# oppo-us-research/PoP-Net

Hardware: AMD Instinct MI355X
Metric: depth-frames/sec end-to-end (480x640) (higher is better)
Workload: dtype bf16

## Files before the change

### popnet_amd/csrc/api.hip

```cpp
#pragma clang fp contract(off)
#include <cmath>
#include <cstdio>
#include <cstdlib>
#include <cstring>
#include "pn_internal.h"
#include "preproc_pixel.h"

template <typename TIN>
__global__ void preprocess_kernel(const TIN *__restrict__ depth, float *__restrict__ out, int B, int H, int W, int S,
                                  double scale_x, double scale_y, float dmax, float mean, float stdv) {
    const unsigned pix = blockIdx.x * blockDim.x + threadIdx.x;
    if (pix >= (unsigned)(S * S)) return;
    const int b = blockIdx.y;
    const int dy = (int)(pix / (unsigned)S);
    const int dx = (int)(pix - (unsigned)dy * (unsigned)S);
    const size_t gid = (size_t)b * S * S + pix;

    out[gid] = pn_preproc_pixel(depth + (size_t)b * H * W, H, W, dy, dx, scale_x, scale_y, dmax, mean, stdv);
}

PnSwitches pn_read_switches() {
    auto set = [](const char *name) { return getenv(name) != nullptr; };
    auto num = [](const char *name, int unset) { const char *e = getenv(name); return e ? atoi(e) : unset; };
    auto is = [](const char *name, const char *value) { const char *e = getenv(name); return e && !strcmp(e, value); };
    PnSwitches s;
    s.no_conv3 = set("POPNET_NO_CONV3");
    s.conv3_rpg8 = set("POPNET_CONV3_RPG8");
    s.conv3_pt14 = num("POPNET_CONV3_PT14", 0);
    s.conv3_nbuf2 = set("POPNET_CONV3_NBUF2");
    s.generic_c64_off = num("POPNET_GENERIC_C64", 1) == 0;
    if (set("POPNET_CONV4")) s.conv4 = num("POPNET_CONV4", 0) == 0 ? 0 : 1;
    s.no_mix = set("POPNET_NO_MIX");
    s.no_bblock = set("POPNET_NO_BBLOCK");
    s.bblock_x3 = num("POPNET_BBLOCK_X3", 0) != 0;
    s.bb64_static = set("POPNET_BB64_STATIC");
    s.bb64_halves = num("POPNET_BB64_HALVES", 1) == 2 ? 2 : 1;
    s.no_tailfuse = set("POPNET_NO_TAILFUSE");
    s.no_poolfuse = set("POPNET_NO_POOLFUSE");
    s.no_stempool = set("POPNET_NO_STEMPOOL");
    s.no_embed3 = set("POPNET_NO_EMBED3");
    s.train_x3_wide = set("POPNET_TRAIN_X3_WIDE");
    s.train_wgrad_novec = set("POPNET_TRAIN_WGRAD_NOVEC");
    s.trainx_one_stream = num("POPNET_TRAINX_STREAMS", 0) == 1;
    s.trainx_stem_handover = set("POPNET_TRAINX_STEM_HANDOVER");
    s.trainx_stem_gather = is("POPNET_TRAINX_STEM_FWD", "gather");
    s.trainx_stem_bn_separate = is("POPNET_TRAINX_STEM_BN", "separate");
    s.trainx_stem_depth = num("POPNET_TRAINX_STEM_DEPTH", 2);
    s.trainx_pack_gather = is("POPNET_TRAINX_PACK", "gather");
    s.trainx_legacy_wgrad = is("POPNET_TRAINX_WGRAD", "legacy");
    return s;
}

extern "C" {

int pn_abi_version(void) { return PN_ABI_VERSION; }
int pn_build_experiments(void) { return 0; }

pn_ctx *pn_create(int device_id) {
    pn_ctx *ctx = new pn_ctx();
    ctx->device = device_id;
    int ndev = 0;
    hipError_t e = hipGetDeviceCount(&ndev);
    if (e != hipSuccess || device_id < 0 || device_id >= ndev) {
        char buf[256];
        snprintf(buf, sizeof buf, "pn_create: device %d not available (%d devices, %s)", device_id, ndev,
                 hipGetErrorString(e));
        ctx->err = buf;
        ctx->device = -1;
        return ctx;
    }
    hipDeviceProp_t prop;
    if (hipGetDeviceProperties(&prop, device_id) == hipSuccess) ctx->num_cus = prop.multiProcessorCount;
    return ctx;
}

void pn_destroy(pn_ctx *ctx) {
    if (!ctx) return;
    if (ctx->parse_ws) (void)hipFree(ctx->parse_ws);
    pn_parse_big_free(ctx);
    if (ctx->train_ws) (void)hipFree(ctx->train_ws);
    for (void *p : ctx->train_ws_retired) (void)hipFree(p);
    for (auto &e : ctx->train_packs) (void)hipFree(e.buf);
    if (ctx->train_pack_table) (void)hipFree(ctx->train_pack_table);
    delete ctx;
}

int pn_last_error(pn_ctx *ctx, char *buf, size_t buf_len) {
    if (!ctx) return 0;
    if (buf && buf_len) {
        size_t n = ctx->err.size() < buf_len - 1 ? ctx->err.size() : buf_len - 1;
        memcpy(buf, ctx->err.data(), n);
// ... 49 lines not shown
```

### popnet_amd/csrc/conv3_kernel.h

```cpp
#pragma once
#include "conv_mfma_kernel.h"

constexpr int PN_CONV3_OCC = 4;
constexpr int PN_CONV3_FAST_EPILOGUE = 2;

__device__ __forceinline__ void pn_glds16(gcptr src, unsigned lds_dst) {
    unsigned keep;
    asm volatile("s_mov_b32 %0, m0\n\ts_mov_b32 m0, %2\n\ts_nop 0\n\tglobal_load_lds_dwordx4 %1, off\n\ts_mov_b32 m0, %0"
                 : "=&s"(keep) : "v"(src), "s"(lds_dst) : "memory");
}

template <int IMM>
__device__ __forceinline__ void pn_glds16_s(const void *sbase, unsigned voff, unsigned lds_dst) {
    unsigned keep;
    asm volatile("s_mov_b32 %0, m0\n\ts_mov_b32 m0, %3\n\ts_nop 0\n\tglobal_load_lds_dwordx4 %1, %2 offset:%4\n\ts_mov_b32 m0, %0"
                 : "=&s"(keep) : "v"(voff), "s"(sbase), "s"(lds_dst), "n"(IMM) : "memory");
}

typedef __attribute__((ext_vector_type(2))) unsigned int u32x2;

template <int KS, int WC, int WP, int NBUF, int PT, int RPG = PT * 4 / 7, int TAIL = 0>
__device__ __forceinline__ void conv3_body(const ConvProblem &P) {
    typedef __bf16 T;
    typedef Elem<PN_PREC_BF16>::Frag Frag;
// ... 403 lines not shown
                    if (cw + k < cout) np[(size_t)k * hw] = v[k];
            }
        }
    };
#define PN3_PIXOF(ba) ((unsigned)(ba) >> 6)
    const int wave_c0 = (cb * WC + wc) * (CT * 16);
    const bool fast = (PN_CONV3_FAST_EPILOGUE == 1 || (PN_CONV3_FAST_EPILOGUE == 2 && WC == 4)) &&
                      wave_c0 + CT * 16 <= cout && P.out && !nchw && !split && !res_split && (act == PN_ACT_RELU || act == PN_ACT_LEAKY || act == PN_ACT_NONE);
    auto finish_fast = [&](auto actc, auto resc) {
        constexpr int ACT = decltype(actc)::value;
        constexpr bool RES = decltype(resc)::value;
        PN_GLOBAL T *ob = (PN_GLOBAL T *)P.out + P.out_coff + wave_c0;
        const PN_GLOBAL T *rb = (const PN_GLOBAL T *)P.res + P.res_coff + wave_c0;
        const unsigned lane_c = (unsigned)(LC * q);
        int ba[PT];
#pragma clang loop unroll(full)
        for (int pt = 0; pt < PT; ++pt) { ba[pt] = baddr[pt]; asm volatile("" : "+v"(ba[pt])); }
        u32x4 rq[PT];
        if (RES) {
#pragma clang loop unroll(full)
            for (int pt = 0; pt < PT; ++pt) {
                const unsigned t = PN3_PIXOF(ba[pt]);
                const unsigned opix = (unsigned)pix0 + (t >> 5) * (unsigned)Wo + (t & 31u);
                rq[pt] = *reinterpret_cast<const PN_GLOBAL u32x4 *>(rb + (opix * (unsigned)res_cs + lane_c));
            }
        }
#pragma clang loop unroll(full)
        for (int pt = 0; pt < PT; ++pt) {
            const int slot = (wp * PT + pt) * 16 + c;
            const unsigned t = PN3_PIXOF(ba[pt]);
            const unsigned opix = (unsigned)pix0 + (t >> 5) * (unsigned)Wo + (t & 31u);
            float v[LC];
#pragma unroll
            for (int ct = 0; ct < CT; ++ct)
#pragma unroll
                for (int i = 0; i < 4; ++i) v[4 * ct + i] = acc[ct][pt][i] + bias[4 * ct + i];
            if (RES) {
                T rv[LC];
                *reinterpret_cast<u32x4 *>(rv) = rq[pt];
#pragma unroll
                for (int k = 0; k < LC; ++k) v[k] += (float)rv[k];
            }
#pragma unroll
            for (int k = 0; k < LC; ++k) {
                if (ACT == PN_ACT_RELU) v[k] = v[k] > 0.f ? v[k] : 0.f;
                else if (ACT == PN_ACT_LEAKY) v[k] = v[k] > 0.f ? v[k] : v[k] * 0.1f;
            }
            T ov[LC];
#pragma unroll
            for (int k = 0; k < LC; ++k) ov[k] = (T)v[k];
            if (slot < npix) *reinterpret_cast<PN_GLOBAL u32x4 *>(ob + (opix * (unsigned)out_cs + lane_c)) = *reinterpret_cast<u32x4 *>(ov);
        }
    };
    if (fast) {
        if (P.res) {
            if (act == PN_ACT_RELU) finish_fast(std::integral_constant<int, PN_ACT_RELU>{}, std::true_type{});
            else if (act == PN_ACT_LEAKY) finish_fast(std::integral_constant<int, PN_ACT_LEAKY>{}, std::true_type{});
            else finish_fast(std::integral_constant<int, PN_ACT_NONE>{}, std::true_type{});
        } else {
            if (act == PN_ACT_RELU) finish_fast(std::integral_constant<int, PN_ACT_RELU>{}, std::false_type{});
            else if (act == PN_ACT_LEAKY) finish_fast(std::integral_constant<int, PN_ACT_LEAKY>{}, std::false_type{});
            else finish_fast(std::integral_constant<int, PN_ACT_NONE>{}, std::false_type{});
        }
        return;
    }
    if (act == PN_ACT_RELU) finish(std::integral_constant<int, PN_ACT_RELU>{});
    else if (act == PN_ACT_LEAKY) finish(std::integral_constant<int, PN_ACT_LEAKY>{});
    else if (act == PN_ACT_NONE) finish(std::integral_constant<int, PN_ACT_NONE>{});
    else finish(std::integral_constant<int, -1>{});
}

template <int KS, int WC, int WP, int NBUF, int PT, int RPG = PT * 4 / 7, int TAIL = 0>
__global__ __launch_bounds__(WC * WP * 64, PT == 14 ? 2 : (NBUF == 2 ? 3 : PN_CONV3_OCC)) void conv3_kernel(const ConvProblem *__restrict__ probs) {
    conv3_body<KS, WC, WP, NBUF, PT, RPG, TAIL>(probs[blockIdx.y]);
}

template <int UNUSED = 0>
__global__ __launch_bounds__(256, PN_CONV3_OCC) void conv3_mix_kernel(const ConvProblem *__restrict__ probs) {
    const ConvProblem &P = probs[blockIdx.y];
    if (P.tail_w) conv3_body<1, 4, 1, 1, 7, 4, 1>(P);
    else if (P.ks == 1) conv3_body<1, 4, 1, 1, 7, 4, 0>(P);
    else conv3_body<3, 4, 1, 1, 7, 4, 0>(P);
}

template <int KS, int WC, int WP, int NBUF, int PT = 7, int RPG = PT * 4 / 7, int TAIL = 0>
static int conv3_launch_one(pn_ctx *ctx, const ConvLaunch &L, hipStream_t stream) {
    auto kern = conv3_kernel<KS, WC, WP, NBUF, PT, RPG, TAIL>;
    if (L.lds_bytes > 48 * 1024) {
        static PnLdsAttr attr;
        if (int rc = pn_lds_attr(ctx, attr, reinterpret_cast<const void *>(kern), L.lds_bytes)) return rc;
    }
    hipLaunchKernelGGL(kern, dim3(L.max_blocks, L.nprob), dim3(WC * WP * 64), L.lds_bytes, stream, L.probs_dev);
    PN_HIP_CHECK(ctx, hipGetLastError());
    return PN_OK;
}
#define PN3_CASE(KS, WC, WP, NB) \
    if (!L.mix && L.ks == KS && L.wc == WC && L.wp == WP && L.nbuf == NB && L.pt == 7 && L.rpg == 4 && !L.tail) return conv3_launch_one<KS, WC, WP, NB>(ctx, L, stream);
#define PN3_CASE_TAIL(KS, WC, WP, NB) \
    if (L.ks == KS && L.wc == WC && L.wp == WP && L.nbuf == NB && L.pt == 7 && L.rpg == 4 && L.tail == 1) return conv3_launch_one<KS, WC, WP, NB, 7, 4, 1>(ctx, L, stream);
#define PN3_CASE_POOLTAIL(KS, WC, WP, NB) \
    if (L.ks == KS && L.wc == WC && L.wp == WP && L.nbuf == NB && L.pt == 7 && L.rpg == 8 && L.tail == 2) return conv3_launch_one<KS, WC, WP, NB, 7, 8, 2>(ctx, L, stream);
#define PN3_CASE_PT(KS, WC, WP, NB, PT_) \
    if (L.ks == KS && L.wc == WC && L.wp == WP && L.nbuf == NB && L.pt == PT_ && L.rpg == PT_ * 4 / 7) return conv3_launch_one<KS, WC, WP, NB, PT_>(ctx, L, stream);
#define PN3_CASE_RPG(KS, WC, WP, NB, RPG_) \
    if (L.ks == KS && L.wc == WC && L.wp == WP && L.nbuf == NB && L.pt == 7 && L.rpg == RPG_) return conv3_launch_one<KS, WC, WP, NB, 7, RPG_>(ctx, L, stream);
int pn_launch_conv3_part0(pn_ctx *ctx, const ConvLaunch &L, hipStream_t stream);
int pn_launch_conv3_part1(pn_ctx *ctx, const ConvLaunch &L, hipStream_t stream);
int pn_launch_conv3_part2(pn_ctx *ctx, const ConvLaunch &L, hipStream_t stream);
```

### popnet_amd/csrc/net.hip

```cpp
#include <cmath>
#include <cstdarg>
#include <cstdio>
#include <algorithm>
#include <cstdlib>
#include <cstring>
#include <map>
#include <memory>
#include <vector>
#include "pn_internal.h"
#include "conv_plan.h"
#include "preproc_pixel.h"

namespace {

struct HostTensor {
    std::vector<int64_t> shape;
    std::vector<float> data;
    size_t numel() const { return data.size(); }
};

struct Buf {
    void *p = nullptr;
    int H = 0, W = 0, C = 0;
    int plane = 0;
};

struct ConvSpec {
    std::string w;
    std::string bn;
    int ks = 3, stride = 1;
    int in_buf = -1, in_coff = 0, cin = 0;
    std::vector<int> cin_map;
    int out_buf = -1, out_coff = 0;
    int res_buf = -1, res_coff = 0;
    int act = PN_ACT_NONE;
    int nchw_slot = -1;
    int cout = 0;
    int cfg = 0, pitch = 0, R = 0, Wt = 0, cin_chunks = 0;
    int kern = 0, wc = 0, wp = 0, nbuf = 0, pt = 7, rpg = 4;
    int wc_min = 0, nbuf_min = 0;
    int k4_level = 0;
    void *wpack = nullptr;
    float *bias = nullptr;
    double flops = 0;
    int tail_conv = -1;
    bool fused_away = false;
    void *tail_wpack = nullptr;
    float *tail_bias = nullptr;
    bool embed3 = false;
    bool pool_tail = false;
    int pool_out_buf = -1, pool_out_coff = 0;
};

struct Step {
    enum Type { STEM, POOL, CONV, BBLOCK } type;
    int bb_a = -1, bb_b = -1, bb_wt = 0;
    void *bb_wpack = nullptr;
    float *bb_bias1 = nullptr, *bb_bias2 = nullptr;
    int *bb_tickets = nullptr;
    bool bb_static = false;
    int bb_halves = 1;
    int out_buf = -1;
    int stem_pool_buf = -1;
    float *stem_w = nullptr, *stem_b = nullptr;
    void *stem_wfrag = nullptr;
    int stem_cin = 1;
    float *stem_scratch = nullptr;
    int mode = 0, in_buf = -1, C = 0, out_coff = 0;
    std::vector<int> conv_ids;
    ConvLaunch launch;
    std::vector<ConvProblem> host_probs;
    ConvProblem *dev_probs = nullptr;
};

uint16_t f32_to_bf16(float f) {
    uint32_t u;
    memcpy(&u, &f, 4);
    if ((u & 0x7fffffffu) > 0x7f800000u) return (uint16_t)((u >> 16) | 0x40);
    u += 0x7fffu + ((u >> 16) & 1u);
    return (uint16_t)(u >> 16);
}

}

struct pn_net {
    pn_ctx *ctx = nullptr;
    int kind = 0, num_parts = 15, a = 14, input_dim = 1;
    std::map<std::string, HostTensor> tensors;
    bool finalized = false;
    int prec = PN_PREC_F32, max_batch = 0, in_h = 0, in_w = 0;
    PnSwitches sw;
    std::vector<Buf> bufs;
    std::vector<ConvSpec> convs;
    std::vector<Step> steps;
    std::vector<void *> dev_allocs;
    float *nchw_ptr[4] = {nullptr, nullptr, nullptr, nullptr};
    int last_B = -1;
    bool x3 = false;
    bool locked = false;
    bool tickets_suspect = false;
    float *last_nchw[4] = {nullptr, nullptr, nullptr, nullptr};
    std::map<std::string, std::pair<int, std::pair<int, int>>> named;
    std::map<std::string, int> named_plane;
    double flops_per_frame = 0;
// ... 444 lines not shown
            }
            if (readers != 1 || other_reader) continue;
            ConvSpec &b = n->convs[ib];
            if (std::find(levels[li + 1].begin(), levels[li + 1].end(), ib) == levels[li + 1].end()) continue;
            const HostTensor *wb = find_t(n, b.w + ".weight");
            if (!wb || wb->shape.size() != 4 || b.ks != 1 || b.stride != 1 || wb->shape[1] != 128 || wb->shape[0] > 32 || !b.bn.empty() || b.res_buf >= 0 || b.in_coff != 0 ||
                (b.act != PN_ACT_NONE && b.act != PN_ACT_SIG && b.act != PN_ACT_SIG_PM2) ||
                !b.cin_map.empty())
                continue;
            a.tail_conv = ib;
            b.fused_away = true;
            a.flops += b.flops;
            levels[li + 1].erase(std::find(levels[li + 1].begin(), levels[li + 1].end(), ib));
        }
    }
    levels.erase(std::remove_if(levels.begin(), levels.end(), [](const std::vector<int> &l) { return l.empty(); }), levels.end());
}


void fuse_pool_tails(pn_net *n, std::vector<std::vector<int>> &levels) {
    if (n->prec != PN_PREC_BF16 || n->sw.no_poolfuse || n->sw.no_conv3) return;
    for (size_t li = 0; li + 1 < levels.size(); ++li) {
        if (levels[li].size() != 1 || levels[li][0] < 0) continue;
        const std::vector<int> &pl = levels[li + 1];
        if (pl.empty() || pl[0] != -1 || pl[1] != 0) continue;
        ConvSpec &a = n->convs[levels[li][0]];
        if (a.kern != 3 || a.ks != 1 || a.stride != 1 || a.cout != 128 || a.wc != 4 || a.wp != 1 || a.res_buf >= 0 || a.nchw_slot >= 0 || a.out_buf < 0 || a.out_coff != 0 ||
            a.tail_conv >= 0 || (a.act != PN_ACT_NONE && a.act != PN_ACT_RELU && a.act != PN_ACT_LEAKY))
            continue;
        if (pl[2] != a.out_buf || pl[4] != 128 || (pl[5] & 7)) continue;
        bool other_reader = false, rewritten = false;
        for (size_t lj = li + 2; lj < levels.size() && !rewritten; ++lj) {
            if (levels[lj].empty()) continue;
            if (levels[lj][0] == -1) {
                if (levels[lj][2] == a.out_buf) other_reader = true;
                if (levels[lj][3] == a.out_buf) rewritten = true;
                continue;
            }
            for (size_t k = levels[lj][0] == -2 ? 1 : 0; k < levels[lj].size(); ++k) {
                const ConvSpec &c = n->convs[levels[lj][k]];
                if (c.in_buf == a.out_buf || c.res_buf == a.out_buf) other_reader = true;
            }
            for (size_t k = levels[lj][0] == -2 ? 1 : 0; k < levels[lj].size(); ++k)
                if (n->convs[levels[lj][k]].out_buf == a.out_buf) rewritten = true;
        }
        if (other_reader) continue;
        a.pool_tail = true;
        a.pool_out_buf = pl[3]; a.pool_out_coff = pl[5];
        a.rpg = 8; a.nbuf = 1;
        levels.erase(levels.begin() + li + 1);
    }
}

int pack_tail(pn_net *n, ConvSpec &a) {
    pn_ctx *ctx = n->ctx;
    const ConvSpec &b = n->convs[a.tail_conv];
    const HostTensor *w = find_t(n, b.w + ".weight"), *bias = find_t(n, b.w + ".bias");
    const int cout = (int)w->shape[0];
    std::vector<uint16_t> pk((size_t)2 * 4 * 64 * 8, 0);
    for (int t = 0; t < 2; ++t)
        for (int ks = 0; ks < 4; ++ks)
            for (int lane = 0; lane < 64; ++lane) {
                const int co = pn_conv_row_channel(t, lane & 15, 2), q = lane >> 4;
                for (int j = 0; j < 8; ++j) {
                    const int ci = ks * 32 + 8 * q + j;
                    pk[(((size_t)t * 4 + ks) * 64 + lane) * 8 + j] = f32_to_bf16(co < cout ? w->data[(size_t)co * 128 + ci] : 0.f);
                }
            }
    if (int rc = dev_alloc(n, &a.tail_wpack, pk.size() * 2, false)) return rc;
    PN_HIP_CHECK(ctx, hipMemcpy(a.tail_wpack, pk.data(), pk.size() * 2, hipMemcpyHostToDevice));
    std::vector<float> hb(32, 0.f);
    for (int o = 0; o < cout; ++o) hb[o] = bias ? bias->data[o] : 0.f;
    if (int rc = dev_alloc(n, (void **)&a.tail_bias, 32 * 4, false)) return rc;
    PN_HIP_CHECK(ctx, hipMemcpy(a.tail_bias, hb.data(), 32 * 4, hipMemcpyHostToDevice));
    return PN_OK;
}

int build_rtpose(pn_net *n) {
    const int H = n->in_h, W = n->in_w;
    if (H % 8 || W % 8) return pn_set_error(n->ctx, PN_ERR_UNSUPPORTED, "input size must be a multiple of 8");
    const int H2 = H / 2, W2 = W / 2, H4 = H / 4, W4 = W / 4, H8 = H / 8, W8 = W / 8;
    const int J1 = n->num_parts + 1, L2 = 2 * n->a, LZ = n->a + 1;
    auto up4 = [](int v) { return (v + 3) / 4 * 4; };
    const int off_paf = 128, off_heat = up4(off_paf + L2), off_z = up4(off_heat + J1);
    const int cat_c = (off_z + LZ + 63) / 64 * 64;
    n->out_h = H8; n->out_w = W8;

    int A1 = new_buf(n, H2, W2, 64), A2 = new_buf(n, H2, W2, 64), T1 = new_buf(n, H2, W2, 64);
    int P1 = new_buf(n, H4, W4, 64), T2 = new_buf(n, H4, W4, 128), D2 = new_buf(n, H4, W4, 128);
    int A3 = new_buf(n, H4, W4, 128), A4 = new_buf(n, H4, W4, 128);
    int CAT = new_buf(n, H8, W8, cat_c);
    int BLa = new_buf(n, H8, W8, 256), BLb = new_buf(n, H8, W8, 256), BLc = new_buf(n, H8, W8, 128);
    int BSa = new_buf(n, H8, W8, 128), BSb = new_buf(n, H8, W8, 128);
    int BDa = new_buf(n, H8, W8, 128), BDb = new_buf(n, H8, W8, 64), BDc = new_buf(n, H8, W8, 64);
    n->named["feat"] = {CAT, {0, 128}};
    n->named["paf1"] = {CAT, {off_paf, L2}};
    n->named["heat1"] = {CAT, {off_heat, J1}};
    n->named["z1"] = {CAT, {off_z, LZ}};

    if (int rc = add_stem(n, A1)) return rc;
    std::vector<std::vector<int>> levels;
    auto level = [&](std::vector<int> ids) { levels.push_back(ids); return 0; };
    level({add_conv(n, "model0.layer1.0.conv1", "model0.layer1.0.bn1", 3, 1, A1, 0, T1, 0, PN_ACT_RELU)});
    level({add_conv(n, "model0.layer1.0.conv2", "model0.layer1.0.bn2", 3, 1, T1, 0, A2, 0, PN_ACT_RELU, A1)});
    level({add_conv(n, "model0.layer1.1.conv1", "model0.layer1.1.bn1", 3, 1, A2, 0, T1, 0, PN_ACT_RELU)});
    level({add_conv(n, "model0.layer1.1.conv2", "model0.layer1.1.bn2", 3, 1, T1, 0, A1, 0, PN_ACT_RELU, A2)});
    levels.push_back({-1, 0, A1, P1, 64, 0});
    level({add_conv(n, "model0.layer2.0.conv1", "model0.layer2.0.bn1", 3, 1, P1, 0, T2, 0, PN_ACT_RELU),
           add_conv(n, "model0.layer2.0.downsample.0", "model0.layer2.0.downsample.1", 1, 1, P1, 0, D2, 0, PN_ACT_NONE)});
    level({add_conv(n, "model0.layer2.0.conv2", "model0.layer2.0.bn2", 3, 1, T2, 0, A3, 0, PN_ACT_RELU, D2)});
    level({add_conv(n, "model0.conv2", "model0.bn2", 1, 1, A3, 0, A4, 0, PN_ACT_RELU)});
    levels.push_back({-1, 0, A4, CAT, 128, 0});

    std::vector<int> map2(cat_c, -1);
    for (int i = 0; i < 128; ++i) map2[i] = L2 + J1 + LZ + i;
    for (int i = 0; i < L2; ++i) map2[off_paf + i] = i;
    for (int i = 0; i < J1; ++i) map2[off_heat + i] = L2 + i;
    for (int i = 0; i < LZ; ++i) map2[off_z + i] = L2 + J1 + i;

    for (int stage = 1; stage <= 2; ++stage) {
        char p1[32], p2[32], p3[32];
        snprintf(p1, sizeof p1, "model%d_1", stage);
        snprintf(p2, sizeof p2, "model%d_2", stage);
        snprintf(p3, sizeof p3, "model%d_3", stage);
        auto nm = [](const char *p, int i) { return std::string(p) + "." + std::to_string(i); };
        std::vector<int> m = stage == 2 ? map2 : std::vector<int>();
        const bool last = stage == 2;
        level({add_conv(n, nm(p1, 0), nm(p1, 1), 3, 1, CAT, 0, BLa, 0, PN_ACT_LEAKY, -1, -1, m),
               add_conv(n, nm(p2, 0), nm(p2, 1), 3, 1, CAT, 0, BSa, 0, PN_ACT_LEAKY, -1, -1, m),
               add_conv(n, nm(p3, 0), nm(p3, 1), 3, 1, CAT, 0, BDa, 0, PN_ACT_LEAKY, -1, -1, m)});
        level({add_conv(n, nm(p1, 3), nm(p1, 4), 3, 1, BLa, 0, BLb, 0, PN_ACT_LEAKY),
               add_conv(n, nm(p2, 3), nm(p2, 4), 3, 1, BSa, 0, BSb, 0, PN_ACT_LEAKY),
               add_conv(n, nm(p3, 3), nm(p3, 4), 3, 1, BDa, 0, BDb, 0, PN_ACT_LEAKY)});
        level({add_conv(n, nm(p1, 6), nm(p1, 7), 3, 1, BLb, 0, BLa, 0, PN_ACT_LEAKY),
               add_conv(n, nm(p2, 6), nm(p2, 7), 3, 1, BSb, 0, BSa, 0, PN_ACT_LEAKY),
               add_conv(n, nm(p3, 6), nm(p3, 7), 3, 1, BDb, 0, BDc, 0, PN_ACT_LEAKY)});
        level({add_conv(n, nm(p1, 9), nm(p1, 10), 1, 1, BLa, 0, BLc, 0, PN_ACT_LEAKY),
               add_conv(n, nm(p2, 9), nm(p2, 10), 3, 1, BSa, 0, BSb, 0, PN_ACT_LEAKY),
               add_conv(n, nm(p3, 9), nm(p3, 10), 3, 1, BDc, 0, BDb, 0, PN_ACT_LEAKY)});
        level({add_conv(n, nm(p1, 12), "", 1, 1, BLc, 0, last ? -1 : CAT, off_paf, PN_ACT_SIG_PM2, -1, last ? 0 : -1),
               add_conv(n, nm(p2, 12), "", 3, 1, BSb, 0, last ? -1 : CAT, off_heat, PN_ACT_SIG, -1, last ? 1 : -1),
               add_conv(n, nm(p3, 12), "", 3, 1, BDb, 0, last ? -1 : CAT, off_z, PN_ACT_SIG_PM2, -1, last ? 2 : -1)});
    }

    for (auto &lv : levels)
        if (lv[0] >= 0) harmonize_level(n, lv);
    for (auto &cs : n->convs)
        if (int rc = prepare_conv(n, cs)) return rc;
    for (auto &cs : n->convs) n->flops_per_frame += cs.flops;
    fuse_basic_blocks(n, levels);
    fuse_1x1_tails(n, levels);
    fuse_pool_tails(n, levels);
    for (auto &cs : n->convs)
        if (cs.tail_conv >= 0)
            if (int rc = pack_tail(n, cs)) return rc;
    for (auto &lv : levels) {
        if (lv[0] == -1) add_pool(n, lv[1], lv[2], lv[3], lv[4], lv[5]);
        else if (lv[0] == -2) { if (int rc = add_bblock(n, lv[1], lv[2])) return rc; }
        else add_conv_level(n, lv);
    }
    return PN_OK;
}

int build_yolo(pn_net *n) {
    const int H = n->in_h, W = n->in_w;
    if (H % 16 || W % 16) return pn_set_error(n->ctx, PN_ERR_UNSUPPORTED, "input size must be a multiple of 16");
    const int H2 = H / 2, W2 = W / 2, H4 = H / 4, W4 = W / 4, H8 = H / 8, W8 = W / 8, H16 = H / 16, W16 = W / 16;
    n->out_h = H16; n->out_w = W16;
    int A1 = new_buf(n, H2, W2, 64);
    int X0 = new_buf(n, H4, W4, 64), X1 = new_buf(n, H4, W4, 64), XT = new_buf(n, H4, W4, 64);
    int Y0 = new_buf(n, H8, W8, 128), Y1 = new_buf(n, H8, W8, 128), YT = new_buf(n, H8, W8, 128), YD = new_buf(n, H8, W8, 128);
    int Na = new_buf(n, H8, W8, 256), Nb = new_buf(n, H8, W8, 256);
    int Ha = new_buf(n, H16, W16, 256), Hb = new_buf(n, H16, W16, 256), Hc = new_buf(n, H16, W16, 128);

    if (int rc = add_stem(n, A1)) return rc;
    std::vector<std::vector<int>> levels;
    auto level = [&](std::vector<int> ids) { levels.push_back(ids); };
    if (n->prec == PN_PREC_BF16 && !n->x3 && n->input_dim == 1 && !n->sw.no_stempool) n->steps.back().stem_pool_buf = X0;
    else levels.push_back({-1, 1, A1, X0, 64, 0});
    int cur = X0, other = X1;
    for (int i = 0; i < 3; ++i) {
        std::string p = "model0.layer1." + std::to_string(i);
        level({add_conv(n, p + ".conv1", p + ".bn1", 3, 1, cur, 0, XT, 0, PN_ACT_RELU)});
        level({add_conv(n, p + ".conv2", p + ".bn2", 3, 1, XT, 0, other, 0, PN_ACT_RELU, cur)});
        std::swap(cur, other);
    }
    {
        const bool embed = n->prec == PN_PREC_BF16 && !n->sw.no_embed3;
        const int c1 = add_conv(n, "model0.layer2.0.conv1", "model0.layer2.0.bn1", 3, 2, cur, 0, YT, 0, PN_ACT_RELU);
        const int cd = add_conv(n, "model0.layer2.0.downsample.0", "model0.layer2.0.downsample.1", embed ? 3 : 1, 2, cur, 0, YD, 0, PN_ACT_NONE);
        n->convs[cd].embed3 = embed;
        level({c1, cd});
    }
    level({add_conv(n, "model0.layer2.0.conv2", "model0.layer2.0.bn2", 3, 1, YT, 0, Y0, 0, PN_ACT_RELU, YD)});
    int yc = Y0, yo = Y1;
    for (int i = 1; i < 4; ++i) {
        std::string p = "model0.layer2." + std::to_string(i);
        level({add_conv(n, p + ".conv1", p + ".bn1", 3, 1, yc, 0, YT, 0, PN_ACT_RELU)});
        level({add_conv(n, p + ".conv2", p + ".bn2", 3, 1, YT, 0, yo, 0, PN_ACT_RELU, yc)});
        std::swap(yc, yo);
    }
    n->named["feat"] = {yc, {0, 128}};
    level({add_conv(n, "model1.0", "model1.1", 3, 1, yc, 0, Na, 0, PN_ACT_LEAKY)});
    level({add_conv(n, "model1.3", "model1.4", 3, 1, Na, 0, Nb, 0, PN_ACT_LEAKY)});
    level({add_conv(n, "model1.6", "model1.7", 3, 1, Nb, 0, Na, 0, PN_ACT_LEAKY)});
// ... 29 lines not shown
            const ConvSpec &cs = n->convs[id];
            const Buf &ib = n->bufs[cs.in_buf];
            ConvProblem P;
            memset(&P, 0, sizeof P);
            const size_t es = n->esize();
            (void)es;
            P.in = ib.p;
            P.wpack = cs.wpack;
            P.bias = cs.bias;
            P.B = B; P.H = ib.H; P.W = ib.W;
            P.Ho = (ib.H + 2 * (cs.ks / 2) - cs.ks) / cs.stride + 1;
            P.Wo = (ib.W + 2 * (cs.ks / 2) - cs.ks) / cs.stride + 1;
            P.cin_chunks = cs.cin_chunks;
            P.in_cs = ib.C; P.in_coff = cs.in_coff;
            if (n->x3 && ib.plane % 64)
                return pn_set_error(n->ctx, PN_ERR_UNSUPPORTED, "bf16x3: input plane of %d channels is not a multiple of 64 (the K loop wraps to the hi plane per 64-channel chunk)", ib.plane);
            P.in_wrap = n->x3 ? 2 * (ib.plane / 64) : (1 << 20);
            P.cout = cs.cout;
            if (cs.out_buf >= 0) { P.out = n->bufs[cs.out_buf].p; P.out_cs = n->bufs[cs.out_buf].C; P.out_coff = cs.out_coff; P.split = n->x3 ? n->bufs[cs.out_buf].plane : 0; }
            if (cs.res_buf >= 0) { P.res = n->bufs[cs.res_buf].p; P.res_cs = n->bufs[cs.res_buf].C; P.res_coff = cs.res_coff; P.res_split = n->x3 ? n->bufs[cs.res_buf].plane : 0; }
            if (cs.nchw_slot >= 0) P.out_nchw = n->nchw_ptr[cs.nchw_slot];
            P.act = cs.act;
            P.yolo_naf = 5 + 3 * n->num_parts;
            P.R = cs.R;
            P.Wt = cs.Wt;
            P.tiles_x = (P.Wo + cs.Wt - 1) / cs.Wt;
            P.tiles_per_img = ((P.Ho + cs.R - 1) / cs.R) * P.tiles_x;
            P.cout_blocks = (cs.cout + BC - 1) / BC;
            P.nblocks = B * P.tiles_per_img * P.cout_blocks;
            if (cs.kern == 4) P.nblocks = ((B * P.tiles_per_img + 1) / 2) * P.cout_blocks;
            P.ksteps = cs.cin_chunks * cs.ks * cs.ks * 2;
            P.ks = cs.ks;
            P.lds_buf_bytes = (int)pn_conv_lds_bytes(n->prec, cs.ks, cs.stride, cs.pitch, cs.R);
            P.lds_two = (cs.cin_chunks > 1 && 2 * (size_t)P.lds_buf_bytes <= 160 * 1024) ? 1 : 0;
            P.in_zero_off = (unsigned)((size_t)n->max_batch * ib.H * ib.W * ib.C * es);
            if (cs.pool_tail) {
                const Buf &pb = n->bufs[cs.pool_out_buf];
                P.tiles_x = (pb.W + 6) / 7;
                P.tiles_per_img = ((pb.H + 2) / 3) * P.tiles_x;
                P.nblocks = B * P.tiles_per_img * P.cout_blocks;
                P.tail_out = pb.p; P.tail_out_cs = pb.C; P.tail_out_coff = cs.pool_out_coff;
                P.tail_split = n->x3 ? pb.plane : 0;
                P.out = nullptr;
                pool_tail = true;
            }
            if (cs.tail_conv >= 0) {
                const ConvSpec &tb = n->convs[cs.tail_conv];
                P.tail_w = cs.tail_wpack; P.tail_bias = cs.tail_bias; P.tail_cout = tb.cout; P.tail_act = tb.act;
                if (tb.out_buf >= 0) { P.tail_out = n->bufs[tb.out_buf].p; P.tail_out_cs = n->bufs[tb.out_buf].C; P.tail_out_coff = tb.out_coff; }
                if (tb.nchw_slot >= 0) P.tail_nchw = n->nchw_ptr[tb.nchw_slot];
                P.out = nullptr;
                has_tail = true;
            }
            if (P.lds_two) two_bufs = true;
            max_blocks = std::max(max_blocks, P.nblocks);
            st.host_probs.push_back(P);
        }
        st.launch.prec = n->prec;
        st.launch.ks = c0.ks; st.launch.stride = c0.stride; st.launch.pitch = c0.pitch; st.launch.cfg = c0.cfg;
        st.launch.nprob = (int)st.host_probs.size();
        st.launch.max_blocks = max_blocks;
        st.launch.lds_bytes = pn_conv_lds_bytes(n->prec, c0.ks, c0.stride, c0.pitch, c0.R) * (two_bufs ? 2 : 1);
        st.launch.kern = c0.kern; st.launch.wc = c0.wc; st.launch.wp = c0.wp; st.launch.nbuf = c0.nbuf; st.launch.pt = c0.pt; st.launch.rpg = c0.rpg;
        if (c0.kern == 3) st.launch.lds_bytes = pn_conv3_lds_bytes(c0.ks, c0.wp, c0.nbuf, c0.rpg);
        st.launch.tail = (c0.kern == 3 && has_tail) ? 1 : (c0.kern == 3 && pool_tail) ? 2 : 0;
        st.launch.mix = 0;
        if (c0.kern == 3) {
            for (int id : st.conv_ids) {
                const ConvSpec &cs = n->convs[id];
                if (cs.ks != c0.ks || (cs.tail_conv >= 0) != (c0.tail_conv >= 0)) st.launch.mix = 1;
                st.launch.lds_bytes = std::max(st.launch.lds_bytes, pn_conv3_lds_bytes(cs.ks, cs.wp, cs.nbuf, cs.rpg));
            }
            if (st.launch.tail == 1) st.launch.lds_bytes = std::max<size_t>(st.launch.lds_bytes, 4 * 7 * 1024 + 1024);
            if (st.launch.tail == 2 && n->x3) st.launch.lds_bytes = std::max<size_t>(st.launch.lds_bytes, 2 * 4 * 7 * 1024);
        }
        if (c0.kern == 4) st.launch.lds_bytes = 0;
        st.launch.probs_dev = st.dev_probs;
        PN_HIP_CHECK(n->ctx, hipMemcpyAsync(st.dev_probs, st.host_probs.data(), st.host_probs.size() * sizeof(ConvProblem),
                                            hipMemcpyHostToDevice, stream));
    }
    n->last_B = B;
    for (int i = 0; i < 4; ++i) n->last_nchw[i] = n->nchw_ptr[i];
    return PN_OK;
}

std::string step_label(const pn_net *n, const Step &st) {
    if (st.type == Step::STEM) {
        if (st.stem_pool_buf >= 0) return "stem7x7_pool_kernel";
        if (st.stem_cin > 1) return "conv2d_forward+nchw_relu_to_nhwc_kernel";
        if (n->prec == PN_PREC_F32) return "stem7x7_kernel";
        return n->x3 ? "stem7x7_mfma_kernel<x3>" : "stem7x7_mfma_kernel";
    }
    if (st.type == Step::POOL) return pn_pool_kernel_label(st.mode, n->x3);
    if (st.type == Step::BBLOCK) return n->x3 ? "bb64x3_kernel" : "bb64_kernel";
    const ConvSpec &c0 = n->convs[st.conv_ids[0]];
    bool mix = false;
    for (int id : st.conv_ids) {
        const ConvSpec &cs = n->convs[id];
        if (cs.ks != c0.ks || (cs.tail_conv >= 0) != (c0.tail_conv >= 0)) mix = true;
    }
    return pn_conv_kernel_label(n->prec, c0.kern, mix, c0.ks, c0.stride, c0.pitch, c0.cfg, c0.wc, c0.wp, c0.nbuf, c0.pt, c0.rpg);
}

int run_forward(pn_net *n, const float *x, int B, hipStream_t stream, int nsteps = -1) {
    pn_ctx *ctx = n->ctx;
    if (!n->finalized) return pn_set_error(ctx, PN_ERR_STATE, "pn_net_finalize has not been called");
    if (B < 1 || B > n->max_batch) return pn_set_error(ctx, PN_ERR_INVALID, "batch %d outside [1, %d]", B, n->max_batch);
    bool dirty = B != n->last_B;
    for (int i = 0; i < 4; ++i) dirty |= n->nchw_ptr[i] != n->last_nchw[i];
    if (dirty) {
        if (n->locked)
            return pn_set_error(ctx, PN_ERR_STATE, "net is locked at batch %d (pn_net_lock): a forward with another batch size or other output buffers would rewrite descriptors a captured graph still reads", n->last_B);
        if (int rc = refresh_problems(n, B, stream)) return rc;
    }
    if (n->tickets_suspect) {
        for (auto &st : n->steps)
            if (st.type == Step::BBLOCK && st.bb_tickets) PN_HIP_CHECK(ctx, hipMemsetAsync(st.bb_tickets, 0, 256, stream));
        n->tickets_suspect = false;
    }
    for (size_t si = 0; si < n->steps.size(); ++si) {
        if ((int)si == nsteps) break;
        Step &st = n->steps[si];
        int rc = PN_OK;
        pn_net::ProfRec *pr = nullptr;
        if (n->profiling) {
            if (n->prof_used == n->prof.size()) {
                pn_net::ProfRec r;
                PN_HIP_CHECK(ctx, hipEventCreate(&r.a));
                PN_HIP_CHECK(ctx, hipEventCreate(&r.b));
                n->prof.push_back(r);
            }
            pr = &n->prof[n->prof_used++];
            pr->kind = (int)st.type;
            pr->flops = 0;
            pr->label.clear();
            if (st.type == Step::CONV) {
                for (int id : st.conv_ids) pr->flops += n->convs[id].flops * B;
                pr->label = step_label(n, st);
            }
            if (st.type == Step::BBLOCK) {
                pr->kind = (int)Step::CONV;
                pr->flops = (n->convs[st.bb_a].flops + n->convs[st.bb_b].flops) * B;
                pr->label = step_label(n, st);
            }
            PN_HIP_CHECK(ctx, hipEventRecord(pr->a, stream));
        }
        if (st.type == Step::STEM && st.stem_pool_buf >= 0) {
            const Buf &ob = n->bufs[st.out_buf], &pb = n->bufs[st.stem_pool_buf];
            rc = pn_launch_stem_pool(ctx, x, st.stem_wfrag, st.stem_b, pb.p, B, n->in_h, n->in_w, ob.H, ob.W, pb.C, stream, n->frame_src.frames ? &n->frame_src : nullptr);
        } else if (st.type == Step::STEM && st.stem_cin > 1) {
            const Buf &ob = n->bufs[st.out_buf];
            if (n->frame_src.frames) return pn_set_error(ctx, PN_ERR_UNSUPPORTED, "the frames-in forward takes single-channel depth frames (input_dim = 1)");
// ... 206 lines not shown
}

int pn_net_num_steps(pn_net *n) {
    if (!n) return PN_ERR_INVALID;
    if (!n->finalized) return pn_set_error(n->ctx, PN_ERR_STATE, "net not finalized");
    return (int)n->steps.size();
}

int pn_net_step_info(pn_net *n, int k, char *out, size_t cap) {
    if (!n || !out || !cap) return PN_ERR_INVALID;
    pn_ctx *ctx = n->ctx;
    if (!n->finalized) return pn_set_error(ctx, PN_ERR_STATE, "net not finalized");
    if (k < -1 || k >= (int)n->steps.size()) return pn_set_error(ctx, PN_ERR_INVALID, "step %d outside [-1, %zu)", k, n->steps.size());
    std::string js;
    char t[256];
    auto add = [&](const char *fmt, ...) {
        va_list ap;
        va_start(ap, fmt);
        vsnprintf(t, sizeof t, fmt, ap);
        va_end(ap);
        js += t;
    };
    auto conv = [&](int id) {
        const ConvSpec &c = n->convs[id];
        add("{\"w\": \"%s\", \"bn\": \"%s\", \"ks\": %d, \"stride\": %d, \"act\": %d, \"cout\": %d, \"embed3\": %d, ",
            c.w.c_str(), c.bn.c_str(), c.embed3 ? 1 : c.ks, c.stride, c.act, c.cout, c.embed3 ? 1 : 0);
        add("\"in_buf\": %d, \"in_coff\": %d, \"res_buf\": %d, \"res_coff\": %d, \"out_buf\": %d, \"out_coff\": %d, \"nchw_slot\": %d, \"cin_map\": [",
            c.in_buf, c.in_coff, c.res_buf, c.res_coff, c.out_buf, c.out_coff, c.nchw_slot);
        for (size_t i = 0; i < c.cin_map.size(); ++i) add(i ? ", %d" : "%d", c.cin_map[i]);
        js += "], \"tail\": ";
        if (c.tail_conv >= 0) {
            const ConvSpec &b = n->convs[c.tail_conv];
            add("{\"w\": \"%s\", \"act\": %d, \"cout\": %d, \"out_buf\": %d, \"out_coff\": %d, \"nchw_slot\": %d}",
                b.w.c_str(), b.act, b.cout, b.out_buf, b.out_coff, b.nchw_slot);
        } else js += "null";
        js += ", \"pool\": ";
        if (c.pool_tail) add("{\"mode\": 0, \"out_buf\": %d, \"out_coff\": %d}", c.pool_out_buf, c.pool_out_coff);
        else js += "null";
        js += "}";
    };
    if (k == -1) {
        add("{\"prec\": \"%s\", \"in_h\": %d, \"in_w\": %d, \"input_dim\": %d, \"max_batch\": %d, \"steps\": %zu, \"bufs\": [",
            n->x3 ? "bf16x3" : n->prec == PN_PREC_BF16 ? "bf16" : "fp32", n->in_h, n->in_w, n->input_dim, n->max_batch, n->steps.size());
        for (size_t i = 0; i < n->bufs.size(); ++i) add(i ? ", [%d, %d, %d]" : "[%d, %d, %d]", n->bufs[i].H, n->bufs[i].W, n->bufs[i].plane);
        js += "]}";
    } else {
        const Step &st = n->steps[k];
        static const char *types[] = {"stem", "pool", "conv", "bblock"};
        add("{\"type\": \"%s\", \"kernel\": \"%s\"", types[(int)st.type], step_label(n, st).c_str());
        if (st.type == Step::STEM) add(", \"cin\": %d, \"out_buf\": %d, \"pool_buf\": %d", st.stem_cin, st.out_buf, st.stem_pool_buf);
        else if (st.type == Step::POOL) add(", \"mode\": %d, \"in_buf\": %d, \"out_buf\": %d, \"C\": %d, \"out_coff\": %d", st.mode, st.in_buf, st.out_buf, st.C, st.out_coff);
        else {
            js += ", \"convs\": [";
            const std::vector<int> ids = st.type == Step::BBLOCK ? std::vector<int>{st.bb_a, st.bb_b} : st.conv_ids;
            for (size_t i = 0; i < ids.size(); ++i) {
                if (i) js += ", ";
                conv(ids[i]);
            }
            js += "]";
        }
        js += "}";
    }
    if (js.size() + 1 > cap) return pn_set_error(ctx, PN_ERR_INVALID, "pn_net_step_info: %zu bytes needed", js.size() + 1);
    memcpy(out, js.c_str(), js.size() + 1);
    return PN_OK;
}

double pn_net_flops_per_frame(pn_net *n) { return n ? n->flops_per_frame : 0.0; }

int pn_net_lock(pn_net *n, int locked) {
    if (!n) return PN_ERR_INVALID;
    if (locked && n->last_B < 0) return pn_set_error(n->ctx, PN_ERR_STATE, "pn_net_lock: run one forward first");
    n->locked = locked != 0;
    return PN_OK;
}

int pn_net_profile_begin(pn_net *n) {
    if (n) n->prof_by_kernel.clear();
    if (!n) return PN_ERR_INVALID;
    n->profiling = true;
    n->prof_used = 0;
    return PN_OK;
}

int pn_net_profile_end(pn_net *n, double *conv_ms, int64_t *conv_launches, double *conv_flops, double *other_ms,
                       int64_t *other_launches) {
    if (!n) return PN_ERR_INVALID;
    pn_ctx *ctx = n->ctx;
    n->profiling = false;
    double cm = 0, om = 0, cf = 0;
    int64_t cl = 0, ol = 0;
    for (size_t i = 0; i < n->prof_used; ++i) {
        PN_HIP_CHECK(ctx, hipEventSynchronize(n->prof[i].b));
        float ms = 0.f;
        PN_HIP_CHECK(ctx, hipEventElapsedTime(&ms, n->prof[i].a, n->prof[i].b));
        if (n->prof[i].kind == (int)Step::CONV) {
            cm += ms; cf += n->prof[i].flops; ++cl;
            auto &e = n->prof_by_kernel[n->prof[i].label];
            e.first.first += ms; e.first.second += 1; e.second += n->prof[i].flops;
        } else { om += ms; ++ol; }
    }
    n->prof_used = 0;
    if (conv_ms) *conv_ms = cm;
    if (conv_launches) *conv_launches = cl;
    if (conv_flops) *conv_flops = cf;
    if (other_ms) *other_ms = om;
    if (other_launches) *other_launches = ol;
// ... 19 lines not shown
```

### popnet_amd/csrc/pn_internal.h

```cpp
#pragma once
#include <hip/hip_runtime.h>
#include <stdint.h>
#include <string>
#include <vector>
#include "../../include/popnet_hip.h"

struct pn_ctx {
    int device = 0;
    std::string err;
    int num_cus = 256;
    void *parse_ws = nullptr;
    size_t parse_ws_bytes = 0;
    bool parse_ws_fixed = false;
    void *parse_big = nullptr;
    void *train_ws = nullptr;
    size_t train_ws_bytes = 0;
    bool train_ws_keep = false;
    std::vector<void *> train_ws_retired;
    bool train_lds_attr = false;
    bool train_x3 = false;
    struct PackEntry { const float *w; int Cout, Cin, flip, x3; void *buf; size_t bytes; bool fresh; };
    bool train_pack_cache = false;
    std::vector<PackEntry> train_packs;
    void *train_pack_table = nullptr;
    size_t train_pack_table_entries = 0;
    size_t train_pack_table_cap = 0;
    unsigned train_pack_blocks = 0;
};

struct PnSwitches {
    bool no_conv3 = false;
    bool conv3_rpg8 = false;
    int conv3_pt14 = 0;
    bool conv3_nbuf2 = false;
    bool generic_c64_off = false;
    int conv4 = -1;
    bool no_mix = false;
    bool no_bblock = false;
    bool bblock_x3 = false;
    bool bb64_static = false;
    int bb64_halves = 1;
    bool no_tailfuse = false;
    bool no_poolfuse = false;
    bool no_stempool = false;
    bool no_embed3 = false;
    bool train_x3_wide = false;
    bool train_wgrad_novec = false;
    bool trainx_one_stream = false;
    bool trainx_stem_handover = false;
    bool trainx_stem_gather = false;
    bool trainx_stem_bn_separate = false;
    int trainx_stem_depth = 2;
    bool trainx_pack_gather = false;
    bool trainx_legacy_wgrad = false;
};
PnSwitches pn_read_switches();

int pn_set_error(pn_ctx *ctx, int code, const char *fmt, ...);
void pn_parse_big_free(pn_ctx *ctx);
int pn_train_ws(pn_ctx *ctx, size_t bytes, void **out);

#define PN_HIP_CHECK(ctx, expr)                                                              \
    do {                                                                                     \
        hipError_t _e = (expr);                                                              \
        if (_e != hipSuccess)                                                                \
            return pn_set_error((ctx), PN_ERR_HIP, "%s failed: %s (%s:%d)", #expr,           \
                                hipGetErrorString(_e), __FILE__, __LINE__);                  \
    } while (0)

struct PnLdsAttr { size_t bytes[64] = {}; };
inline int pn_lds_attr(pn_ctx *ctx, PnLdsAttr &st, const void *kern, size_t bytes) {
    const int d = ctx->device >= 0 && ctx->device < 64 ? ctx->device : 0;
    if (st.bytes[d] >= bytes) return PN_OK;
    PN_HIP_CHECK(ctx, hipFuncSetAttribute(kern, hipFuncAttributeMaxDynamicSharedMemorySize, (int)bytes));
    st.bytes[d] = bytes;
    return PN_OK;
}

enum pn_act {
    PN_ACT_NONE = 0,
    PN_ACT_RELU = 1,
    PN_ACT_LEAKY = 2,
    PN_ACT_SIG_PM2 = 3,
    PN_ACT_SIG = 4,
    PN_ACT_YOLO = 5
};

struct ConvProblem {
    const void *in;
    const void *wpack;
    const float *bias;
    const void *res;
    void *out;
    float *out_nchw;
    int B, H, W;
    int Ho, Wo;
    int cin_chunks;
    int in_cs, in_coff;
    int cout;
    int out_cs, out_coff;
    int res_cs, res_coff;
    int act;
    int yolo_naf;
    int R;
    int Wt, tiles_x;
    int tiles_per_img;
    int cout_blocks;
    int nblocks;
    int ksteps;
    int ks;
    int lds_buf_bytes;
    int lds_two;
    unsigned in_zero_off;
    int split;
    int res_split;
    int in_wrap;
    const void *tail_w;
    const float *tail_bias;
    void *tail_out;
    float *tail_nchw;
    int tail_cout, tail_act, tail_out_cs, tail_out_coff;
    int tail_split;
};

enum pn_conv_cfg {
    PN_CFG_C128 = 0,
    PN_CFG_C64 = 1,
    PN_CFG_C32 = 2,
    PN_CFG_C16 = 3,
    PN_CFG_C64W = 4
};
int pn_cfg_couts(int cfg);
inline int pn_cfg_ct(int cfg) { return cfg == PN_CFG_C16 ? 1 : 2; }
inline int pn_conv_row_channel(int tile, int row, int CT) {
    return (tile / CT) * CT * 16 + 4 * CT * (row >> 2) + 4 * (tile % CT) + (row & 3);
}
int pn_cfg_pixels(int cfg);

struct ConvLaunch {
    int prec;
    int ks;
    int stride;
    int pitch;
    int cfg;
    int kern = 0, wc = 0, wp = 0, nbuf = 0, pt = 7, rpg = 4;
    int tail = 0;
    int mix = 0;
    int nprob;
    int max_blocks;
    size_t lds_bytes;
    const ConvProblem *probs_dev;
};
int pn_launch_conv(pn_ctx *ctx, const ConvLaunch &L, hipStream_t stream);
inline std::string pn_conv_kernel_label(int prec, int kern, bool mix, int ks, int stride, int pitch, int cfg, int wc, int wp, int nbuf, int pt, int rpg) {
    char lb[96];
    if (kern == 4) snprintf(lb, sizeof lb, "conv4_kernel");
    else if (kern == 3 && mix) snprintf(lb, sizeof lb, "conv3_mix_kernel");
    else if (kern == 3) snprintf(lb, sizeof lb, "conv3_kernel<%d, %d, %d, %d, %d, %d>", ks, wc, wp, nbuf, pt, rpg);
    else snprintf(lb, sizeof lb, "conv_mfma_kernel<%d, %d, %d, %d, %d>", prec, ks, stride, pitch, cfg);
    return lb;
}
inline std::string pn_pool_kernel_label(int mode, bool split) {
    char lb[48];
    snprintf(lb, sizeof lb, "pool_kernel<%d%s>", mode, split ? ", split" : "");
    return lb;
}
int pn_launch_conv3(pn_ctx *ctx, const ConvLaunch &L, hipStream_t stream);
int pn_launch_conv4(pn_ctx *ctx, const ConvLaunch &L, hipStream_t stream);

struct BBProblem {
    const void *in;
    void *out;
    const void *wpack;
    const float *bias1, *bias2;
    int B, H, W;
// ... 36 lines not shown
```

Baseline: 69290.

## Fuse sibling 1x1 conv into 3x3 conv3 block sharing the same input tile

Adds a TAIL==3 variant of the conv3 body. After the 3x3 conv finishes its epilogue, the same block computes a sibling 1x1 conv over the centre tap of the input tile it already has in LDS, then writes that result to the sibling's output buffer. A planner pass pairs eligible 3x3/1x1 convs in the same level that read the same input, removing one input read and one block's work from the launch. In exchange, the fused blocks do more serial work and hold more register pressure, which may hurt occupancy or load balance.

```diff
diff --git a/popnet_amd/csrc/api.hip b/popnet_amd/csrc/api.hip
--- a/popnet_amd/csrc/api.hip
+++ b/popnet_amd/csrc/api.hip
@@ -37,6 +37,7 @@
     s.bb64_halves = num("POPNET_BB64_HALVES", 1) == 2 ? 2 : 1;
     s.no_tailfuse = set("POPNET_NO_TAILFUSE");
     s.no_poolfuse = set("POPNET_NO_POOLFUSE");
+    s.no_sibfuse = set("POPNET_NO_SIBFUSE");
     s.no_stempool = set("POPNET_NO_STEMPOOL");
     s.no_embed3 = set("POPNET_NO_EMBED3");
     s.train_x3_wide = set("POPNET_TRAIN_X3_WIDE");
diff --git a/popnet_amd/csrc/conv3_kernel.h b/popnet_amd/csrc/conv3_kernel.h
--- a/popnet_amd/csrc/conv3_kernel.h
+++ b/popnet_amd/csrc/conv3_kernel.h
@@ -479,6 +479,11 @@
             if (slot < npix) *reinterpret_cast<PN_GLOBAL u32x4 *>(ob + (opix * (unsigned)out_cs + lane_c)) = *reinterpret_cast<u32x4 *>(ov);
         }
     };
+    if constexpr (TAIL == 3) {
+        if (act == PN_ACT_RELU) finish_fast(std::integral_constant<int, PN_ACT_RELU>{}, std::false_type{});
+        else if (act == PN_ACT_LEAKY) finish_fast(std::integral_constant<int, PN_ACT_LEAKY>{}, std::false_type{});
+        else finish_fast(std::integral_constant<int, PN_ACT_NONE>{}, std::false_type{});
+    } else {
     if (fast) {
         if (P.res) {
             if (act == PN_ACT_RELU) finish_fast(std::integral_constant<int, PN_ACT_RELU>{}, std::true_type{});
@@ -495,6 +500,68 @@
     else if (act == PN_ACT_LEAKY) finish(std::integral_constant<int, PN_ACT_LEAKY>{});
     else if (act == PN_ACT_NONE) finish(std::integral_constant<int, PN_ACT_NONE>{});
     else finish(std::integral_constant<int, -1>{});
+    }
+
+    if constexpr (TAIL == 3) {
+        static_assert(KS == 3 && WC == 4 && WP == 1 && NBUF == 1 && PT == 7 && RPG == 4, "the carried sibling is built for the one-chunk 128-cout 3x3 block");
+        const __amdgpu_buffer_rsrc_t srs = __builtin_amdgcn_make_buffer_rsrc(const_cast<void *>(P.sib_w), 0, 0x7fffffff, 0x00020000);
+        unsigned slane = (unsigned)lane * 16u;
+        asm volatile("" : "+v"(slane));
+        Frag a2[2][CT];
+#pragma unroll
+        for (int s = 0; s < 2; ++s)
+#pragma unroll
+            for (int ct = 0; ct < CT; ++ct)
+                a2[s][ct] = __builtin_bit_cast(Frag, __builtin_amdgcn_raw_buffer_load_b128(srs, slane, (unsigned)__builtin_amdgcn_readfirstlane(((wc * CT + ct) * 2 + s) * FRAGB), 0));
+#pragma unroll
+        for (int ct = 0; ct < CT; ++ct)
+#pragma unroll
+            for (int pt = 0; pt < PT; ++pt) acc[ct][pt] = f32x4{0.f, 0.f, 0.f, 0.f};
+        constexpr int CENTRE = (PITCH + 1) * 64;
+        int sa[PT];
+#pragma clang loop unroll(full)
+        for (int pt = 0; pt < PT; ++pt) { sa[pt] = baddr[pt]; asm volatile("" : "+v"(sa[pt])); }
+#pragma clang loop unroll(full)
+        for (int s = 0; s < 2; ++s)
+#pragma clang loop unroll(full)
+            for (int pt = 0; pt < PT; ++pt) {
+                const Frag bf = read_b_frag<PN_PREC_BF16>(smem + s * (IMG / 2) + CENTRE, sa[pt]);
+#pragma unroll
+                for (int ct = 0; ct < CT; ++ct) acc[ct][pt] = mma(a2[s][ct], bf, acc[ct][pt]);
+            }
+        float sbias[LC];
+#pragma unroll
+        for (int ct = 0; ct < CT; ++ct) {
+            const f32x4 b4 = *reinterpret_cast<const PN_GLOBAL f32x4 *>((const PN_GLOBAL float *)P.sib_bias + cw + 4 * ct);
+            sbias[4 * ct + 0] = b4[0]; sbias[4 * ct + 1] = b4[1]; sbias[4 * ct + 2] = b4[2]; sbias[4 * ct + 3] = b4[3];
+        }
+        PN_GLOBAL T *sob = (PN_GLOBAL T *)P.sib_out + P.sib_out_coff + wave_c0 + LC * q;
+        const unsigned sib_cs = (unsigned)P.sib_out_cs;
+        auto finish_sib = [&](auto actc) {
+            constexpr int ACT = decltype(actc)::value;
+#pragma clang loop unroll(full)
+            for (int pt = 0; pt < PT; ++pt) {
+                const int slot = pt * 16 + c;
+                const unsigned t = PN3_PIXOF(sa[pt]);
+                const unsigned opix = (unsigned)pix0 + (t >> 5) * (unsigned)Wo + (t & 31u);
+                T ov[LC];
+#pragma unroll
+                for (int ct = 0; ct < CT; ++ct)
+#pragma unroll
+                    for (int i = 0; i < 4; ++i) {
+                        float v = acc[ct][pt][i] + sbias[4 * ct + i];
+                        if (ACT == PN_ACT_RELU) v = v > 0.f ? v : 0.f;
+                        else if (ACT == PN_ACT_LEAKY) v = v > 0.f ? v : v * 0.1f;
+                        ov[4 * ct + i] = (T)v;
+                    }
+                if (slot < npix) *reinterpret_cast<PN_GLOBAL u32x4 *>(sob + opix * sib_cs) = *reinterpret_cast<u32x4 *>(ov);
+            }
+        };
+        const int sact = P.sib_act;
+        if (sact == PN_ACT_RELU) finish_sib(std::integral_constant<int, PN_ACT_RELU>{});
+        else if (sact == PN_ACT_LEAKY) finish_sib(std::integral_constant<int, PN_ACT_LEAKY>{});
+        else finish_sib(std::integral_constant<int, PN_ACT_NONE>{});
+    }
 }
 
 template <int KS, int WC, int WP, int NBUF, int PT, int RPG = PT * 4 / 7, int TAIL = 0>
@@ -506,6 +573,7 @@
 __global__ __launch_bounds__(256, PN_CONV3_OCC) void conv3_mix_kernel(const ConvProblem *__restrict__ probs) {
     const ConvProblem &P = probs[blockIdx.y];
     if (P.tail_w) conv3_body<1, 4, 1, 1, 7, 4, 1>(P);
+    else if (P.sib_w) conv3_body<3, 4, 1, 1, 7, 4, 3>(P);
     else if (P.ks == 1) conv3_body<1, 4, 1, 1, 7, 4, 0>(P);
     else conv3_body<3, 4, 1, 1, 7, 4, 0>(P);
 }
diff --git a/popnet_amd/csrc/net.hip b/popnet_amd/csrc/net.hip
--- a/popnet_amd/csrc/net.hip
+++ b/popnet_amd/csrc/net.hip
@@ -50,6 +50,7 @@
     bool embed3 = false;
     bool pool_tail = false;
     int pool_out_buf = -1, pool_out_coff = 0;
+    int sib_conv = -1;
 };
 
 struct Step {
@@ -600,6 +601,34 @@
     }
 }
 
+void fuse_1x1_siblings(pn_net *n, std::vector<std::vector<int>> &levels) {
+    if (n->prec != PN_PREC_BF16 || n->x3 || n->sw.no_sibfuse || n->sw.no_mix || n->sw.no_conv3) return;
+    for (auto &lv : levels) {
+        if (lv.empty() || lv[0] < 0) continue;
+        for (size_t ia = 0; ia < lv.size(); ++ia) {
+            ConvSpec &a = n->convs[lv[ia]];
+            if (a.kern != 3 || a.ks != 3 || a.stride != 1 || a.cout != 128 || a.wc != 4 || a.wp != 1 || a.nbuf != 1 || a.pt != 7 || a.rpg != 4 || a.cin_chunks != 1 ||
+                a.tail_conv >= 0 || a.pool_tail || a.sib_conv >= 0 || a.embed3 || a.res_buf >= 0 || a.nchw_slot >= 0 || a.out_buf < 0 || (a.out_coff & 7) ||
+                (n->bufs[a.out_buf].C & 7) || (a.act != PN_ACT_NONE && a.act != PN_ACT_RELU && a.act != PN_ACT_LEAKY))
+                continue;
+            for (size_t ib = 0; ib < lv.size(); ++ib) {
+                ConvSpec &b = n->convs[lv[ib]];
+                if (ib == ia || b.kern != 3 || b.ks != 1 || b.stride != 1 || b.cout != 128 || b.wc != 4 || b.wp != 1 || b.nbuf != 1 || b.pt != 7 || b.rpg != 4 || b.cin_chunks != 1 ||
+                    b.tail_conv >= 0 || b.pool_tail || b.embed3 || b.res_buf >= 0 || b.nchw_slot >= 0 || b.out_buf < 0 || (b.out_coff & 7) || (n->bufs[b.out_buf].C & 7) ||
+                    (b.act != PN_ACT_NONE && b.act != PN_ACT_RELU && b.act != PN_ACT_LEAKY))
+                    continue;
+                if (b.in_buf != a.in_buf || b.in_coff != a.in_coff || b.R != a.R || b.Wt != a.Wt) continue;
+                a.sib_conv = lv[ib];
+                b.fused_away = true;
+                a.flops += b.flops;
+                lv.erase(lv.begin() + ib);
+                break;
+            }
+            if (a.sib_conv >= 0) break;
+        }
+    }
+}
+
 int pack_tail(pn_net *n, ConvSpec &a) {
     pn_ctx *ctx = n->ctx;
     const ConvSpec &b = n->convs[a.tail_conv];
@@ -699,6 +728,7 @@
     fuse_basic_blocks(n, levels);
     fuse_1x1_tails(n, levels);
     fuse_pool_tails(n, levels);
+    fuse_1x1_siblings(n, levels);
     for (auto &cs : n->convs)
         if (cs.tail_conv >= 0)
             if (int rc = pack_tail(n, cs)) return rc;
@@ -834,6 +864,11 @@
                 P.out = nullptr;
                 has_tail = true;
             }
+            if (cs.sib_conv >= 0) {
+                const ConvSpec &sb = n->convs[cs.sib_conv];
+                P.sib_w = sb.wpack; P.sib_bias = sb.bias; P.sib_act = sb.act;
+                P.sib_out = n->bufs[sb.out_buf].p; P.sib_out_cs = n->bufs[sb.out_buf].C; P.sib_out_coff = sb.out_coff;
+            }
             if (P.lds_two) two_bufs = true;
             max_blocks = std::max(max_blocks, P.nblocks);
             st.host_probs.push_back(P);
@@ -850,7 +885,7 @@
         if (c0.kern == 3) {
             for (int id : st.conv_ids) {
                 const ConvSpec &cs = n->convs[id];
-                if (cs.ks != c0.ks || (cs.tail_conv >= 0) != (c0.tail_conv >= 0)) st.launch.mix = 1;
+                if (cs.ks != c0.ks || (cs.tail_conv >= 0) != (c0.tail_conv >= 0) || cs.sib_conv >= 0) st.launch.mix = 1;
                 st.launch.lds_bytes = std::max(st.launch.lds_bytes, pn_conv3_lds_bytes(cs.ks, cs.wp, cs.nbuf, cs.rpg));
             }
             if (st.launch.tail == 1) st.launch.lds_bytes = std::max<size_t>(st.launch.lds_bytes, 4 * 7 * 1024 + 1024);
@@ -879,7 +914,7 @@
     bool mix = false;
     for (int id : st.conv_ids) {
         const ConvSpec &cs = n->convs[id];
-        if (cs.ks != c0.ks || (cs.tail_conv >= 0) != (c0.tail_conv >= 0)) mix = true;
+        if (cs.ks != c0.ks || (cs.tail_conv >= 0) != (c0.tail_conv >= 0) || cs.sib_conv >= 0) mix = true;
     }
     return pn_conv_kernel_label(n->prec, c0.kern, mix, c0.ks, c0.stride, c0.pitch, c0.cfg, c0.wc, c0.wp, c0.nbuf, c0.pt, c0.rpg);
 }
@@ -1192,7 +1227,10 @@
         else if (st.type == Step::POOL) add(", \"mode\": %d, \"in_buf\": %d, \"out_buf\": %d, \"C\": %d, \"out_coff\": %d", st.mode, st.in_buf, st.out_buf, st.C, st.out_coff);
         else {
             js += ", \"convs\": [";
-            const std::vector<int> ids = st.type == Step::BBLOCK ? std::vector<int>{st.bb_a, st.bb_b} : st.conv_ids;
+            std::vector<int> ids = st.type == Step::BBLOCK ? std::vector<int>{st.bb_a, st.bb_b} : st.conv_ids;
+            if (st.type == Step::CONV)
+                for (int id : st.conv_ids)
+                    if (n->convs[id].sib_conv >= 0) ids.push_back(n->convs[id].sib_conv);
             for (size_t i = 0; i < ids.size(); ++i) {
                 if (i) js += ", ";
                 conv(ids[i]);
diff --git a/popnet_amd/csrc/pn_internal.h b/popnet_amd/csrc/pn_internal.h
--- a/popnet_amd/csrc/pn_internal.h
+++ b/popnet_amd/csrc/pn_internal.h
@@ -42,6 +42,7 @@
     int bb64_halves = 1;
     bool no_tailfuse = false;
     bool no_poolfuse = false;
+    bool no_sibfuse = false;
     bool no_stempool = false;
     bool no_embed3 = false;
     bool train_x3_wide = false;
@@ -121,6 +122,10 @@
     float *tail_nchw;
     int tail_cout, tail_act, tail_out_cs, tail_out_coff;
     int tail_split;
+    const void *sib_w;
+    const float *sib_bias;
+    void *sib_out;
+    int sib_act, sib_out_cs, sib_out_coff;
 };
 
 enum pn_conv_cfg {
```

After: 69760, median of 6. About the same (+0.7%).
